# pqpeqr/RL-2048-with-Reinforce-and-Actor-Critic

Hardware: AMD Instinct MI355X
Metric: env steps/sec (whole node) + achieved HBM GB/s, batch=1M 4x4 boards (higher is better)
Workload: dtype u64

## Files before the change

### rl-2048-with-reinforce-and-actor-critic_amd/csrc/g2048.hip

```cpp
#include <hip/hip_runtime.h>

#include <cstdlib>
#include <mutex>
#include <string>

#include "g2048.h"
#include "g2048_core.h"

using namespace g2048;

static_assert(G2048_F_CHANGED == kFChanged && G2048_F_TERMINATED == kFTerminated && G2048_F_TRUNCATED == kFTruncated &&
                  G2048_F_INVALID == kFInvalid && G2048_F_OVERFLOW == kFOverflow,
              "g2048_core.h step flag bits == include/g2048.h");

namespace {

thread_local std::string g_err;
std::mutex g_mu;
constexpr int kMaxDev = 64;
uint8_t* g_tab[kMaxDev] = {};
int g_cus[kMaxDev] = {};

int fail(int code, const std::string& msg) {
    g_err = msg;
    return code;
}

#define G2048_HIP(x)                                                                                  \
    do {                                                                                              \
        hipError_t e_ = (x);                                                                          \
        if (e_ != hipSuccess) return fail(G2048_EHIP, std::string(#x) + ": " + hipGetErrorString(e_)); \
    } while (0)

#ifndef G2048_DIAG
#define G2048_DIAG 0
#endif
#if G2048_DIAG
constexpr int kDiagSlots = 5, kDiagBlocks = 4096;
__device__ uint64_t g_diag_ts[kDiagBlocks * kDiagSlots];
#define G2048_TS(slot)                                                                          \
    do {                                                                                        \
        if (threadIdx.x == 0 && blockIdx.x < kDiagBlocks)                                       \
            g_diag_ts[blockIdx.x * kDiagSlots + (slot)] = __builtin_amdgcn_s_memrealtime();     \
    } while (0)
#else
#define G2048_TS(slot) \
    do {               \
    } while (0)
#endif

constexpr int kBlock = 1024;
constexpr int kLines = 65536;
constexpr int kTabBytes = kLines * 2 + kLines / 2;
constexpr int kTabVec = kTabBytes / 16;
constexpr int kMxOff = kTabBytes;
constexpr int kDevTabBytes = kTabBytes + kLines / 2;
constexpr int kLutSmallN = 16384;
constexpr int64_t kMaxLanesPerLaunch = int64_t(1) << 27;

template <class T>
__device__ __forceinline__ T ld(const T* p, uint32_t idx) {
    return *reinterpret_cast<const T*>(reinterpret_cast<const char*>(p) + idx * (uint32_t)sizeof(T));
}
template <class T>
__device__ __forceinline__ void st(T* p, uint32_t idx, T v) {
    *reinterpret_cast<T*>(reinterpret_cast<char*>(p) + idx * (uint32_t)sizeof(T)) = v;
}

__device__ __forceinline__ void st_obs(float4* base, int q, float4 v) {
    typedef float f4v __attribute__((ext_vector_type(4)));
    __builtin_nontemporal_store(f4v{v.x, v.y, v.z, v.w}, reinterpret_cast<f4v*>(base + q));
}

struct LineFn {
    const uint16_t* line;
    __device__ uint32_t operator()(uint32_t o) const { return line[o]; }
};
struct CodeFn {
    const uint8_t* code;
    __device__ uint32_t operator()(uint32_t o) const { return (code[o >> 1] >> ((o & 1u) << 2)) & 15u; }
};

__device__ inline uint64_t shfl64(uint64_t v, int src) {
    uint32_t lo = (uint32_t)__shfl((int)(uint32_t)v, src, 64);
    uint32_t hi = (uint32_t)__shfl((int)(uint32_t)(v >> 32), src, 64);
    return ((uint64_t)hi << 32) | lo;
}

__device__ inline uint32_t nib(uint64_t b, uint32_t cell) { return (uint32_t)(b >> (4u * cell)) & 15u; }

template <int OBS>
__device__ inline void write_obs_wave(float* __restrict__ obs, uint32_t w0, uint64_t b, uint64_t wmask, int lane,
                                      float scale) {
    if constexpr (OBS == G2048_OBS_ONEHOT) {
        float4* dst = reinterpret_cast<float4*>(obs) + (size_t)w0 * 68;
        const auto value = [&](int q, int src, uint64_t bb) {
            const int j = (q - src * 68) * 4;
            const int c0 = j / 17;
            const int c1 = c0 + 1 < 16 ? c0 + 1 : 15;
            const int p0 = 17 * c0 + (int)nib(bb, c0);
            const int p1 = 17 * c1 + (int)nib(bb, c1);
            float4 v;
            v.x = (j == p0 || j == p1) ? 1.0f : 0.0f;
            v.y = (j + 1 == p0 || j + 1 == p1) ? 1.0f : 0.0f;
            v.z = (j + 2 == p0 || j + 2 == p1) ? 1.0f : 0.0f;
            v.w = (j + 3 == p0 || j + 3 == p1) ? 1.0f : 0.0f;
            return v;
        };
        if (wmask == ~0ull) {
#pragma unroll 4
            for (int k = 0; k < 68; k++) {
                const int q = k * 64 + lane;
                const int src = q / 68;
                st_obs(dst, q, value(q, src, shfl64(b, src)));
            }
        } else {
#pragma unroll 4
            for (int k = 0; k < 68; k++) {
                const int q = k * 64 + lane;
                const int src = q / 68;
                const uint64_t bb = shfl64(b, src);
// ... 72 lines not shown
    g.i_hi = c.y;
    g.has_uint32 = 0u;
    g.uinteger = ld(L.rng_uint, i);
    return g;
}

__device__ inline void store_pcg(const g2048_lanes& L, uint32_t i, const Pcg64& g, bool with_inc) {
    st(reinterpret_cast<ulonglong2*>(L.rng_state), i, make_ulonglong2(g.s_lo, g.s_hi));
    if (with_inc) st(reinterpret_cast<ulonglong2*>(L.rng_inc), i, make_ulonglong2(g.i_lo, g.i_hi));
    st(L.rng_uint, i, g.uinteger);
}

__device__ inline uint32_t fresh_state(const Pcg64& g) {
    return (2u << G2048_LS_MAXT_SHIFT) | G2048_LS_ACTIVE | (g.has_uint32 ? G2048_LS_HAS_U32 : 0u);
}

__device__ inline U4 philox_ctr(uint64_t key, uint64_t seed, uint32_t ctr, uint32_t tag) {
    U4 c{(uint32_t)seed, (uint32_t)(seed >> 32), ctr, tag};
    return philox4x32(c, (uint32_t)key, (uint32_t)(key >> 32));
}

template <int RNG>
__device__ inline uint64_t fresh_board(uint64_t seed, uint64_t key, Pcg64& g) {
    uint64_t b = 0;
    if constexpr (RNG == G2048_RNG_PCG64) {
        g = pcg_seed(seed);
        b = spawn_pcg(b, g);
        b = spawn_pcg(b, g);
    } else {
        const U4 r = philox_ctr(key, seed, 0u, 1u);
        b = spawn_philox(b, U4{r.x, r.y, 0u, 0u});
        b = spawn_philox(b, U4{r.z, r.w, 0u, 0u});
    }
    return b;
}

struct StepArgs {
    g2048_lanes L;
    const uint8_t* actions;
    g2048_step_out out;
    RewardCfg rc;
    float obs_scale;
    int auto_reset;
    int64_t max_steps;
    uint64_t stride, key;
    const uint8_t* tab;
    uint32_t n;
    int diag;
};

template <int OBS, int RNG>
__device__ inline void reset_lane(const StepArgs& a, uint32_t i, uint64_t prev_seed) {
    const g2048_lanes& L = a.L;
    const uint64_t seed = prev_seed + a.stride;
    Pcg64 g;
    g.has_uint32 = 0u;
    const uint64_t b = fresh_board<RNG>(seed, a.key, g);
    st(L.seed, i, seed);
    st(L.board, i, b);
    st(L.state, i, fresh_state(g));
    if constexpr (RNG == G2048_RNG_PCG64) store_pcg(L, i, g, true);
    if (a.out.mask) st(reinterpret_cast<uint32_t*>(a.out.mask), i, mask_word(action_mask(b)));
    if (a.out.mask_bits) st(a.out.mask_bits, i, (uint8_t)action_mask(b));
    if constexpr (OBS != G2048_OBS_NONE)
        if (a.out.obs) write_obs_lane<OBS>(a.out.obs, i, b, a.obs_scale);
}

struct LaneIn {
    uint64_t b, seed;
    uint32_t st, act;
    Pcg64 g;
};

template <int RNG>
__device__ inline void load_lane(const StepArgs& a, uint32_t i, LaneIn& x) {
    const g2048_lanes& L = a.L;
    x.b = ld(L.board, i);
    x.st = ld(L.state, i);
    x.act = ld(a.actions, i);
    if constexpr (RNG == G2048_RNG_PCG64) x.g = load_pcg(L, i);
    else x.seed = ld(L.seed, i);
}

template <int RNG, int XO, int RK>
__device__ inline uint64_t step_lane(const StepArgs& a, uint32_t i, LaneIn& x, const LineFn& lut,
                                     const CodeFn& code, bool& wobs, bool& reset, uint32_t& mbits) {
    static_assert(RK == 0 || XO == 0 || XO == 3, "the lean path writes no score / merged list");
    constexpr bool LIST = XO == 2, EXTRA = XO == 1 || XO == 2;
    const g2048_lanes& L = a.L;
    const uint64_t b = x.b;
    if (EXTRA && a.out.prev_board) st(a.out.prev_board, i, b);
    wobs = false;
    reset = false;
    if (!(x.st & G2048_LS_ACTIVE) || x.act > 3u) {
        st(a.out.reward, i, 0.0f);
        if (EXTRA && a.out.reward64) st(a.out.reward64, i, 0.0);
        st(a.out.flags, i, (uint8_t)((x.st & G2048_LS_ACTIVE) ? G2048_F_BADACTION : G2048_F_INACTIVE));
        if (LIST && a.out.merged) st(a.out.merged, i, 0u);
        if (EXTRA && a.out.score_add) st(a.out.score_add, i, 0u);
        return b;
    }
    const uint32_t sc0 = x.st & G2048_LS_STEP_MASK;
    const uint32_t sc = sc0 + (sc0 < G2048_LS_STEP_MASK ? 1u : 0u);
    uint32_t mt = (x.st >> G2048_LS_MAXT_SHIFT) & 31u;
    if constexpr (RNG == G2048_RNG_PCG64) x.g.has_uint32 = (x.st & G2048_LS_HAS_U32) ? 1u : 0u;

    MoveSummary s;
    uint64_t m, nzm = 0;
    if (G2048_DIAG && (a.diag & 4)) {
        s = MoveSummary{0, 0, 0, 0, 0, 0};
        m = b ^ ((uint64_t)x.act << 60);
        nzm = nz_bits(m);
    } else if constexpr (RK == 1) {
        m = board_move_lean(b, x.act, lut, code, s, nzm);
    } else {
        m = board_move_coded<LIST>(b, x.act, lut, code, s);
    }
    const bool changed = m != b;
    if constexpr (RK == 1) {
        if constexpr (RNG == G2048_RNG_PCG64) {
            if (!(G2048_DIAG && (a.diag & 4))) {
                Pcg64 g2 = x.g;
                uint64_t nzbit;
                const uint64_t m2 = spawn_pcg_lean(m, ~nzm & kNibLsb, g2, nzbit);
                m = changed ? m2 : m;
                nzm = changed ? nzm | nzbit : nzm;
                x.g.s_hi = changed ? g2.s_hi : x.g.s_hi;
                x.g.s_lo = changed ? g2.s_lo : x.g.s_lo;
                x.g.uinteger = changed ? g2.uinteger : x.g.uinteger;
                x.g.has_uint32 = changed ? g2.has_uint32 : x.g.has_uint32;
            }
        } else if (changed && !(G2048_DIAG && (a.diag & 4))) {
            uint64_t nzbit;
            m = spawn_philox_z(m, ~nzm & kNibLsb, philox_ctr(a.key, x.seed, sc, 0u), nzbit);
            nzm |= nzbit;
        }
    } else {
        if (changed && !(G2048_DIAG && (a.diag & 4))) {
            if constexpr (RNG == G2048_RNG_PCG64) m = spawn_pcg(m, x.g);
            else m = spawn_philox(m, philox_ctr(a.key, x.seed, sc, 0u));
        }
        nzm = nz_bits(m);
    }
    const BoardBits bits = board_bits_nz(m, nzm);
    const bool done = bits_done(bits);
    const bool invalid = !changed && !done;
    const double r = env_reward_nz<RK == 1>(a.rc, s, nzm, done, invalid, mt);
    const bool trunc = a.max_steps >= 0 && (int64_t)sc >= a.max_steps && !done;
    const uint32_t fl = (changed ? G2048_F_CHANGED : 0u) | (done ? G2048_F_TERMINATED : 0u) |
                        (trunc ? G2048_F_TRUNCATED : 0u) | (invalid ? G2048_F_INVALID : 0u) |
                        (s.overflow ? G2048_F_OVERFLOW : 0u);
    st(a.out.reward, i, (float)r);
    if (EXTRA && a.out.reward64) st(a.out.reward64, i, r);
    if (LIST && a.out.merged) st(a.out.merged, i, s.list);
    if (EXTRA && a.out.score_add) st(a.out.score_add, i, s.score);
    reset = (done || trunc) && a.auto_reset;
    uint32_t nst = sc | (mt << G2048_LS_MAXT_SHIFT) | ((done || trunc) ? 0u : G2048_LS_ACTIVE);
    if constexpr (RNG == G2048_RNG_PCG64) nst |= x.g.has_uint32 ? G2048_LS_HAS_U32 : 0u;
    st(a.out.flags, i, (uint8_t)(fl | (reset ? G2048_F_RESET : 0u)));
    st(L.board, i, m);
    st(L.state, i, nst);
    if constexpr (RNG == G2048_RNG_PCG64) store_pcg(L, i, x.g, false);
    wobs = true;
    mbits = bits_mask(bits);
    return m;
}

template <int OBS, int RNG, int XO, int RK>
__device__ __forceinline__ void sweep(const StepArgs& a, uint32_t w0, int lane, LaneIn& x, const LineFn& lut,
                                      const CodeFn& code, uint64_t& pending, uint64_t& pseed, uint32_t k) {
    const uint32_t i = w0 + lane;
    bool wobs = false, reset = false;
    uint32_t mbits = 0;
    uint64_t b = 0;
    if (i < a.n) b = step_lane<RNG, XO, RK>(a, i, x, lut, code, wobs, reset, mbits);
    if (reset) {
        if (!pending) {
            if constexpr (RNG == G2048_RNG_PCG64) pseed = ld(a.L.seed, i);
            else pseed = x.seed;
        }
        pending |= 1ull << k;
    }
    if constexpr (XO == 3) {
        if (wobs) st(a.out.mask_bits, i, (uint8_t)mbits);
    } else {
        if (wobs && a.out.mask) st(reinterpret_cast<uint32_t*>(a.out.mask), i, mask_word(mbits));
        if (wobs && a.out.mask_bits) st(a.out.mask_bits, i, (uint8_t)mbits);
    }
    if constexpr (OBS != G2048_OBS_NONE) {
        const uint64_t wm = __ballot(wobs);
        if (G2048_DIAG && (a.diag & 16)) return;
        if (a.out.obs && wm) write_obs_wave<OBS>(a.out.obs, w0, b, wm, lane, a.obs_scale);
    }
}

constexpr int kStepLdsBytes = kTabBytes;
constexpr int kStepLdsVec = kStepLdsBytes / 16;
constexpr int kResetCap = (kStepLdsBytes - 16) / 12;
static_assert(16 + kResetCap * 4 + kResetCap * 8 <= kStepLdsBytes, "reset list fits the LDS area");
static_assert(kTabVec % kBlock == 0, "table fill: whole chunks per thread");

template <int OBS, int RNG, bool LDS, int XO, int U, int RK>
__global__ void __launch_bounds__(kBlock) step_kernel(StepArgs a) {
    static_assert(U == 1, "one board per lane per sweep");
    __shared__ uint4 tab_lds[LDS ? kStepLdsVec : 1];
    const int lane = threadIdx.x & 63;
    const uint32_t w_first = (blockIdx.x * kBlock + threadIdx.x) & ~63u;
    const uint32_t wstride = gridDim.x * kBlock;
    const uint32_t wend = a.n;
    const uint32_t last = a.n - 1u;
    const auto lane_at = [&](uint32_t w) { return w + lane < last ? w + lane : last; };
    G2048_TS(0);
    LaneIn A, B, C;
    uint32_t w0 = w_first, w1 = w_first + wstride;
    load_lane<RNG>(a, lane_at(w0), A);
    load_lane<RNG>(a, lane_at(w1), B);
    const uint8_t* tab = a.tab;
    if constexpr (LDS) {
        const uint4* src = reinterpret_cast<const uint4*>(a.tab);
        if (!(G2048_DIAG && (a.diag & 1))) {
            constexpr uint32_t kChunks = kTabVec / kBlock;
            const uint32_t rot = blockIdx.x % kChunks;
#pragma unroll
            for (uint32_t j = 0; j < kChunks; j++) {
                uint32_t c = j + rot;
                c -= c >= kChunks ? kChunks : 0u;
                const uint32_t k = c * kBlock + threadIdx.x;
                tab_lds[k] = src[k + (RK == 1 && c >= 8u ? (uint32_t)((kMxOff - 2 * kLines) / 16) : 0u)];
            }
        }
        __syncthreads();
        tab = reinterpret_cast<const uint8_t*>(tab_lds);
    }
    G2048_TS(1);
    const LineFn lut{reinterpret_cast<const uint16_t*>(tab)};
    const CodeFn code{tab + (LDS || RK == 0 ? 2 * kLines : kMxOff)};
    uint64_t pending = 0, pseed = 0;
    uint32_t k = 0;
    while (w0 < wend) {
        const uint32_t w2 = w1 + wstride;
        load_lane<RNG>(a, lane_at(w2), C);
        sweep<OBS, RNG, XO, RK>(a, w0, lane, A, lut, code, pending, pseed, k);
        if (w1 >= wend) break;
        const uint32_t w3 = w2 + wstride;
        load_lane<RNG>(a, lane_at(w3), A);
        sweep<OBS, RNG, XO, RK>(a, w1, lane, B, lut, code, pending, pseed, k + 1);
        if (w2 >= wend) break;
        const uint32_t w4 = w3 + wstride;
        load_lane<RNG>(a, lane_at(w4), B);
        sweep<OBS, RNG, XO, RK>(a, w2, lane, C, lut, code, pending, pseed, k + 2);
        w0 = w3;
        w1 = w4;
        k += 3;
    }
    if (G2048_DIAG && (a.diag & 2)) pending = 0;
    if constexpr (LDS) {
        uint32_t* cnt = reinterpret_cast<uint32_t*>(tab_lds);
        uint32_t* ridx = cnt + 4;
        uint64_t* rseed = reinterpret_cast<uint64_t*>(ridx + kResetCap + (kResetCap & 1));
        __syncthreads();
        G2048_TS(2);
        if (threadIdx.x == 0) *cnt = 0u;
        __syncthreads();
        bool first = true;
        while (__ballot(pending != 0ull)) {
            const bool has = pending != 0ull;
            const uint32_t kk = has ? (uint32_t)__builtin_ctzll(pending) : 0u;
            const uint32_t i = w_first + kk * wstride + lane;
            const uint64_t sd = first ? pseed : (has ? ld(a.L.seed, i) : 0ull);
            const uint64_t bal = __ballot(has);
            const int leader = __builtin_ctzll(bal);
            uint32_t base = 0;
            if (lane == leader) base = atomicAdd(cnt, (uint32_t)__popcll(bal));
            base = (uint32_t)__shfl((int)base, leader, 64);
            const uint32_t slot =
                base + __builtin_amdgcn_mbcnt_hi((uint32_t)(bal >> 32), __builtin_amdgcn_mbcnt_lo((uint32_t)bal, 0u));
            if (has) {
                if (slot < (uint32_t)kResetCap) {
                    ridx[slot] = i;
                    rseed[slot] = sd;
                } else {
                    reset_lane<OBS, RNG>(a, i, sd);
                }
                pending &= pending - 1ull;
            }
            first = false;
        }
        __syncthreads();
        G2048_TS(3);
        const uint32_t R = *cnt < (uint32_t)kResetCap ? *cnt : (uint32_t)kResetCap;
        for (uint32_t r = threadIdx.x; r < R; r += kBlock) reset_lane<OBS, RNG>(a, ridx[r], rseed[r]);
    } else {
        bool first = true;
        while (pending) {
            const uint32_t kk = (uint32_t)__builtin_ctzll(pending);
            pending &= pending - 1ull;
            const uint32_t i = w_first + kk * wstride + lane;
            reset_lane<OBS, RNG>(a, i, first ? pseed : ld(a.L.seed, i));
            first = false;
        }
    }
#if G2048_DIAG
    __syncthreads();
    G2048_TS(4);
#endif
}

struct ResetArgs {
    g2048_lanes L;
    const uint64_t* seeds;
    const uint8_t* reset_mask;
    int8_t* mask_out;
    float* obs_out;
    float obs_scale;
    uint64_t key;
    uint32_t n;
};

template <int OBS, int RNG>
__global__ void __launch_bounds__(256) reset_kernel(ResetArgs a) {
    const int lane = threadIdx.x & 63;
    const uint32_t w_first = (blockIdx.x * blockDim.x + threadIdx.x) & ~63u;
    const uint32_t wstride = gridDim.x * blockDim.x;
    for (uint32_t w0 = w_first; w0 < a.n; w0 += wstride) {
        const uint32_t i = w0 + lane;
        bool w = false;
        uint64_t b = 0;
        if (i < a.n && (!a.reset_mask || ld(a.reset_mask, i))) {
            const uint64_t seed = a.seeds ? ld(a.seeds, i) : ld(a.L.seed, i);
            Pcg64 g;
            g.has_uint32 = 0u;
            b = fresh_board<RNG>(seed, a.key, g);
            st(a.L.seed, i, seed);
            st(a.L.board, i, b);
            st(a.L.state, i, fresh_state(g));
            if constexpr (RNG == G2048_RNG_PCG64) store_pcg(a.L, i, g, true);
// ... 502 lines not shown
```

### rl-2048-with-reinforce-and-actor-critic_amd/csrc/g2048_core.h

```cpp
#pragma once
#include <math.h>
#include <stdint.h>

#ifdef __HIPCC__
#define G2048_HD __host__ __device__ inline
#else
#define G2048_HD static inline
#endif

namespace g2048 {

constexpr uint64_t kNibLsb = 0x1111111111111111ull;
constexpr uint64_t kHMask = 0x0111011101110111ull;
constexpr uint64_t kVMask = 0x0000111111111111ull;

G2048_HD int popc64(uint64_t x) { return __builtin_popcountll(x); }

G2048_HD uint64_t nz_bits(uint64_t b) {
    uint64_t x = b | (b >> 1);
    x |= x >> 2;
    return x & kNibLsb;
}

G2048_HD uint64_t transpose(uint64_t x) {
// ... 238 lines not shown
}

G2048_HD uint32_t line_move_alu(uint32_t o, uint32_t& e0, uint32_t& e1) {
    uint32_t out = 0u, sh = 0u, pend = o & 15u;
    e0 = 0u;
    e1 = 0u;
#pragma unroll
    for (int k = 1; k < 4; k++) {
        const uint32_t v = bfe32(o, 4u * k, 4u);
        const bool nz = v != 0u;
        const bool mg = nz && v == pend;
        const uint32_t emit = mg ? (v == 15u ? 15u : v + 1u) : (nz ? pend : 0u);
        out |= emit << sh;
        sh += emit != 0u ? 4u : 0u;
        e1 = (mg && e0 != 0u) ? v + 1u : e1;
        e0 = (mg && e0 == 0u) ? v + 1u : e0;
        pend = mg ? 0u : (nz ? v : pend);
    }
    return out | (pend << sh);
}

template <bool WANT_LIST>
G2048_HD uint64_t board_move_alu(uint64_t b, uint32_t a, MoveSummary& s) {
    const uint64_t mvert = 0ull - (uint64_t)((a == 0u) | (a == 2u));
    const uint64_t mrev = 0ull - (uint64_t)((a == 1u) | (a == 2u));
    const bool back = (a == 0u) | (a == 1u);
    uint64_t f = b ^ ((b ^ transpose(b)) & mvert);
    f ^= (f ^ reverse_rows(f)) & mrev;
    uint32_t e0[4], e1[4];
    uint64_t g = 0;
    uint32_t sum_e = 0, score = 0, max_e = 0, count = 0, list = 0;
#pragma unroll
    for (int j = 0; j < 4; j++) {
        const uint32_t nw = line_move_alu((uint32_t)(f >> (16 * j)) & 0xFFFFu, e0[j], e1[j]);
        g |= (uint64_t)nw << (16 * j);
        score += ((1u << e0[j]) & ~1u) + ((1u << e1[j]) & ~1u);
        sum_e += e0[j] + e1[j];
        max_e = max_e > e0[j] ? max_e : e0[j];
        max_e = max_e > e1[j] ? max_e : e1[j];
    }
    if (WANT_LIST) {
#pragma unroll
        for (int jj = 0; jj < 4; jj++) {
            const uint32_t x0 = back ? e0[3 - jj] : e0[jj], x1 = back ? e1[3 - jj] : e1[jj];
            const uint32_t n0 = x0 != 0u, n1 = x1 != 0u;
            if (n0) list |= ((x0 - 1u) & 15u) << (4u * (count & 7u));
            if (n1) list |= ((x1 - 1u) & 15u) << (4u * ((count + n0) & 7u));
            count += n0 + n1;
        }
    } else {
#pragma unroll
        for (int j = 0; j < 4; j++) count += (e0[j] != 0u) + (e1[j] != 0u);
    }
    s.count = count;
    s.sum_e = sum_e;
    s.score = score;
    s.max_e = max_e;
    s.overflow = max_e >> 4;
    s.list = list;
    g ^= (g ^ reverse_rows(g)) & mrev;
    g ^= (g ^ transpose(g)) & mvert;
    return g;
}

G2048_HD uint32_t line_max_merge_field(uint32_t row) {
    uint32_t e0, e1;
    (void)line_move_alu(row, e0, e1);
    const uint32_t m = e0 > e1 ? e0 : e1;
    return m ? m - 1u : 0u;
}

G2048_HD uint32_t nib_sum64(uint64_t x) {
    const uint64_t t = (x & 0x0F0F0F0F0F0F0F0Full) + ((x >> 4) & 0x0F0F0F0F0F0F0F0Full);
#ifdef __HIP_DEVICE_COMPILE__
    return __builtin_amdgcn_sad_u8((uint32_t)t, 0u, __builtin_amdgcn_sad_u8((uint32_t)(t >> 32), 0u, 0u));
#else
    uint64_t y = t + (t >> 8);
    y += y >> 16;
    y += y >> 32;
    return (uint32_t)(y & 0xFFu);
#endif
}

template <class Lut, class Mx>
G2048_HD uint64_t board_move_lean(uint64_t b, uint32_t a, const Lut& lut, const Mx& mx, MoveSummary& s,
                                  uint64_t& nzg) {
    const uint64_t mvert = 0ull - (uint64_t)((a == 0u) | (a == 2u));
    const uint64_t mrev = 0ull - (uint64_t)((a == 1u) | (a == 2u));
    uint64_t f = b ^ ((b ^ transpose(b)) & mvert);
    f ^= (f ^ reverse_rows(f)) & mrev;
    uint32_t o[4], nw[4], fm[4];
#pragma unroll
    for (int j = 0; j < 4; j++) o[j] = (uint32_t)(f >> (16 * j)) & 0xFFFFu;
#pragma unroll
    for (int j = 0; j < 4; j++) {
        nw[j] = (uint32_t)lut(o[j]);
        fm[j] = (uint32_t)mx(o[j]);
    }
    uint64_t g = 0;
#pragma unroll
    for (int j = 0; j < 4; j++) g |= (uint64_t)nw[j] << (16 * j);
    const uint32_t m01 = fm[0] > fm[1] ? fm[0] : fm[1], m23 = fm[2] > fm[3] ? fm[2] : fm[3];
    const uint32_t mf = m01 > m23 ? m01 : m23;
    g ^= (g ^ reverse_rows(g)) & mrev;
    g ^= (g ^ transpose(g)) & mvert;
    nzg = nz_bits(g);
    s.max_e = mf ? mf + 1u : 0u;
    s.overflow = mf == 15u;
    s.count = (uint32_t)(popc64(nz_bits(b)) - popc64(nzg));
    s.sum_e = nib_sum64(b) - nib_sum64(g) + 2u * s.count;
    if (s.overflow) {
        uint32_t se = 0;
#pragma unroll
        for (int j = 0; j < 4; j++) {
            const LineMerges m = line_merges(o[j], nw[j]);
            se += m.e0 + m.e1;
        }
        s.sum_e = se;
    }
    s.score = 0u;
    s.list = 0u;
    return g;
}

struct BoardBits {
    uint64_t nz, z, eqh, eqv;
};

G2048_HD BoardBits board_bits_nz(uint64_t b, uint64_t nz) {
    BoardBits r;
    r.nz = nz;
    r.z = ~r.nz & kNibLsb;
    r.eqh = ~nz_bits(b ^ (b >> 4)) & r.nz & kHMask;
    r.eqv = ~nz_bits(b ^ (b >> 16)) & r.nz & kVMask;
    return r;
}

G2048_HD BoardBits board_bits(uint64_t b) { return board_bits_nz(b, nz_bits(b)); }

G2048_HD bool bits_done(const BoardBits& r) { return r.z == 0 && (r.eqh | r.eqv) == 0; }

G2048_HD uint32_t bits_mask(const BoardBits& r) {
    uint32_t up = ((r.z & (r.nz >> 16) & kVMask) | r.eqv) != 0;
    uint32_t down = ((r.nz & (r.z >> 16) & kVMask) | r.eqv) != 0;
    uint32_t left = ((r.z & (r.nz >> 4) & kHMask) | r.eqh) != 0;
    uint32_t right = ((r.nz & (r.z >> 4) & kHMask) | r.eqh) != 0;
    return up | (right << 1) | (down << 2) | (left << 3);
}

G2048_HD uint32_t kth_empty_cell(uint64_t zbits, uint32_t k) {
    uint32_t pos = 0;
    uint32_t c = (uint32_t)popc64(zbits & 0xFFFFFFFFull);
    if (k >= c) { k -= c; zbits >>= 32; pos += 32; }
    c = (uint32_t)popc64(zbits & 0xFFFFull);
    if (k >= c) { k -= c; zbits >>= 16; pos += 16; }
    c = (uint32_t)popc64(zbits & 0xFFull);
    if (k >= c) { k -= c; zbits >>= 8; pos += 8; }
    c = (uint32_t)popc64(zbits & 0xFull);
    if (k >= c) { pos += 4; }
    return pos >> 2;
}

struct Pcg64 {
    uint64_t s_lo, s_hi, i_lo, i_hi;
    uint32_t has_uint32, uinteger;
};

constexpr uint64_t kPcgMulHi = 0x2360ED051FC65DA4ull;
constexpr uint64_t kPcgMulLo = 0x4385DF649FCCF645ull;

G2048_HD uint64_t mulhi64(uint64_t a, uint64_t b) { return (uint64_t)(((unsigned __int128)a * b) >> 64); }

G2048_HD void pcg_step(Pcg64& g) {
    uint64_t lo = g.s_lo * kPcgMulLo;
    uint64_t hi = mulhi64(g.s_lo, kPcgMulLo) + g.s_lo * kPcgMulHi + g.s_hi * kPcgMulLo;
    uint64_t nlo = lo + g.i_lo;
    g.s_hi = hi + g.i_hi + (nlo < lo);
    g.s_lo = nlo;
}

G2048_HD uint64_t pcg_next64(Pcg64& g) {
    pcg_step(g);
    uint64_t x = g.s_hi ^ g.s_lo;
    uint32_t rot = (uint32_t)(g.s_hi >> 58);
    return (x >> rot) | (x << ((64u - rot) & 63u));
}

G2048_HD uint32_t pcg_next32(Pcg64& g) {
    if (g.has_uint32) {
        g.has_uint32 = 0;
        return g.uinteger;
    }
    uint64_t v = pcg_next64(g);
    g.has_uint32 = 1;
    g.uinteger = (uint32_t)(v >> 32);
    return (uint32_t)v;
}

G2048_HD double pcg_random(Pcg64& g) { return (double)(pcg_next64(g) >> 11) * (1.0 / 9007199254740992.0); }

G2048_HD uint32_t pcg_bounded(Pcg64& g, uint32_t n) {
    if (n <= 1u) return 0u;
    const uint32_t rng = n - 1u;
    uint64_t m = (uint64_t)pcg_next32(g) * n;
    uint32_t left = (uint32_t)m;
// ... 22 lines not shown

G2048_HD Pcg64 pcg_seed(uint64_t seed) {
    const uint32_t w0 = (uint32_t)seed, w1 = (uint32_t)(seed >> 32);
    const bool two = w1 != 0u;
    uint32_t pool[4];
    uint32_t hc = 0x43b0d7e5u;
    pool[0] = ss_hashmix(w0, hc);
    pool[1] = ss_hashmix(two ? w1 : 0u, hc);
    pool[2] = ss_hashmix(0u, hc);
    pool[3] = ss_hashmix(0u, hc);
#pragma unroll
    for (int s = 0; s < 4; s++)
#pragma unroll
        for (int d = 0; d < 4; d++)
            if (s != d) pool[d] = ss_mix(pool[d], ss_hashmix(pool[s], hc));
    uint32_t w[8];
    uint32_t hb = 0x8b51f9ddu;
#pragma unroll
    for (int i = 0; i < 8; i++) {
        uint32_t v = pool[i & 3];
        v ^= hb;
        hb *= 0x58f38dedu;
        v *= hb;
        v ^= v >> 16;
        w[i] = v;
    }
    const uint64_t st_hi = ((uint64_t)w[1] << 32) | w[0], st_lo = ((uint64_t)w[3] << 32) | w[2];
    const uint64_t sq_hi = ((uint64_t)w[5] << 32) | w[4], sq_lo = ((uint64_t)w[7] << 32) | w[6];
    Pcg64 g;
    g.i_hi = (sq_hi << 1) | (sq_lo >> 63);
    g.i_lo = (sq_lo << 1) | 1u;
    g.s_lo = 0;
    g.s_hi = 0;
    pcg_step(g);
    uint64_t lo = g.s_lo + st_lo;
    g.s_hi = g.s_hi + st_hi + (lo < g.s_lo);
    g.s_lo = lo;
    pcg_step(g);
    g.has_uint32 = 0;
    g.uinteger = 0;
    return g;
}

struct U4 {
    uint32_t x, y, z, w;
};

G2048_HD U4 philox4x32(U4 c, uint32_t k0, uint32_t k1) {
#pragma unroll
    for (int r = 0; r < 10; r++) {
        const uint64_t p0 = (uint64_t)0xD2511F53u * c.x;
        const uint64_t p1 = (uint64_t)0xCD9E8D57u * c.z;
        U4 n;
        n.x = (uint32_t)(p1 >> 32) ^ c.y ^ k0;
        n.y = (uint32_t)p1;
        n.z = (uint32_t)(p0 >> 32) ^ c.w ^ k1;
        n.w = (uint32_t)p0;
        c = n;
        k0 += 0x9E3779B9u;
        k1 += 0xBB67AE85u;
    }
    return c;
}

G2048_HD uint64_t spawn_pcg_z(uint64_t b, uint64_t z, Pcg64& g, uint64_t& nzbit) {
    nzbit = 0;
    uint32_t n = (uint32_t)popc64(z);
    if (n == 0u) return b;
    uint32_t k = pcg_bounded(g, n);
    uint32_t cell = kth_empty_cell(z, k);
    uint64_t e = pcg_random(g) < 0.9 ? 1u : 2u;
    nzbit = 1ull << (4u * cell);
    return b | (e << (4u * cell));
}

G2048_HD uint64_t pcg_output(uint64_t s_hi, uint64_t s_lo) {
    const uint64_t x = s_hi ^ s_lo;
    const uint32_t rot = (uint32_t)(s_hi >> 58);
    return (x >> rot) | (x << ((64u - rot) & 63u));
}

constexpr uint64_t kRandom09 = 8106479329266893ull;

G2048_HD uint64_t spawn_pcg_lean(uint64_t b, uint64_t z, Pcg64& g, uint64_t& nzbit) {
    const uint32_t n = (uint32_t)popc64(z);
    Pcg64 A = g;
    pcg_step(A);
    Pcg64 B = A;
    pcg_step(B);
    const uint64_t oA = pcg_output(A.s_hi, A.s_lo);
    const bool draw = n > 1u;
    const bool fresh = draw && !g.has_uint32;
    const uint32_t u = g.has_uint32 ? g.uinteger : (uint32_t)oA;
    const uint64_t m = (uint64_t)u * n;
    if (draw && (uint32_t)m < n) return spawn_pcg_z(b, z, g, nzbit);
    const uint32_t k = draw ? (uint32_t)(m >> 32) : 0u;
    const uint64_t r_hi = fresh ? B.s_hi : A.s_hi, r_lo = fresh ? B.s_lo : A.s_lo;
    const uint64_t e = (pcg_output(r_hi, r_lo) >> 11) < kRandom09 ? 1u : 2u;
    const uint32_t cell = kth_empty_cell(z, k);
    g.s_hi = r_hi;
    g.s_lo = r_lo;
    g.uinteger = fresh ? (uint32_t)(oA >> 32) : g.uinteger;
    g.has_uint32 = draw ? (g.has_uint32 ^ 1u) : g.has_uint32;
    nzbit = 1ull << (4u * cell);
    return b | (e << (4u * cell));
}

G2048_HD uint64_t spawn_pcg(uint64_t b, Pcg64& g) {
    uint64_t nzbit;
    return spawn_pcg_z(b, ~nz_bits(b) & kNibLsb, g, nzbit);
}

G2048_HD uint32_t softmax_select(const float lg[4], uint32_t mw, bool has_mask, bool greedy, double u, float p[4]) {
    const bool m[4] = {(mw & 0xFFu) != 0u, ((mw >> 8) & 0xFFu) != 0u, ((mw >> 16) & 0xFFu) != 0u, (mw >> 24) != 0u};
    float l[4];
    for (int k = 0; k < 4; k++) l[k] = (!has_mask || m[k]) ? lg[k] : -1e9f;
    const float mx = fmaxf(fmaxf(l[0], l[1]), fmaxf(l[2], l[3]));
    float e[4];
    for (int k = 0; k < 4; k++) e[k] = expf(l[k] - mx);
    const float s = ((e[0] + e[1]) + e[2]) + e[3];
    for (int k = 0; k < 4; k++) p[k] = e[k] / s;
    uint32_t act = 0;
    if (greedy) {
        float best = has_mask ? p[0] * (float)m[0] : p[0];
        for (int k = 1; k < 4; k++) {
            const float q = has_mask ? p[k] * (float)m[k] : p[k];
            if (q > best) {
                best = q;
                act = (uint32_t)k;
            }
        }
    } else {
        double cdf[4], acc = 0.0;
        for (int k = 0; k < 4; k++) {
            acc += (double)p[k];
            cdf[k] = acc;
        }
        for (int k = 0; k < 4; k++) act += (cdf[k] / cdf[3] <= u) ? 1u : 0u;
    }
    return act;
}

G2048_HD uint64_t spawn_philox_z(uint64_t b, uint64_t z, U4 r, uint64_t& nzbit) {
    nzbit = 0;
    uint32_t n = (uint32_t)popc64(z);
    if (n == 0u) return b;
    uint32_t k = (uint32_t)(((uint64_t)r.x * n) >> 32);
    uint32_t cell = kth_empty_cell(z, k);
    uint64_t e = r.y < 3865470566u ? 1u : 2u;
    nzbit = 1ull << (4u * cell);
    return b | (e << (4u * cell));
}

G2048_HD uint64_t spawn_philox(uint64_t b, U4 r) {
    uint64_t nzbit;
    return spawn_philox_z(b, ~nz_bits(b) & kNibLsb, r, nzbit);
}

struct RewardCfg {
    int32_t reward_mode, bonus_mode, use_action_mask;
    uint32_t terms;
    double base_reward_scale, empty_tile_reward, merge_reward, bonus_scale, step_reward, endgame_penalty,
        invalid_action_penalty;
};

constexpr uint32_t kRwInvalidPenalty = 1u, kRwLog2 = 2u, kRwEmpty = 4u, kRwMerge = 8u, kRwEndgame = 16u,
                   kRwBonusRaw = 32u, kRwBonusLog2 = 64u;
G2048_HD uint32_t reward_terms(const RewardCfg& c) {
    return (c.use_action_mask ? 0u : kRwInvalidPenalty) | (c.reward_mode == 0 ? 0u : kRwLog2) |
           (c.empty_tile_reward != 0.0 ? kRwEmpty : 0u) | (c.merge_reward != 0.0 ? kRwMerge : 0u) |
           (c.endgame_penalty != 0.0 ? kRwEndgame : 0u) | (c.bonus_mode == 1 ? kRwBonusRaw : 0u) |
           (c.bonus_mode == 2 ? kRwBonusLog2 : 0u);
}

template <bool LOG2_ONLY = false>
G2048_HD double env_reward_nz(const RewardCfg& c, const MoveSummary& s, uint64_t final_nz, bool done, bool invalid,
                              uint32_t& max_tile_e) {
    uint32_t t = c.terms;
#ifdef __HIP_DEVICE_COMPILE__
    asm volatile("" : "+s"(t));
#endif
    if ((t & kRwInvalidPenalty) && invalid) return c.invalid_action_penalty;
    double r = (LOG2_ONLY || (t & kRwLog2)) ? (double)s.sum_e : (double)s.score;
    r *= c.base_reward_scale;
    if (t & kRwEmpty) {
        const int ne = 16 - popc64(final_nz);
        r += c.empty_tile_reward * (double)ne;
    }
// ... 65 lines not shown
```

Before: 33.65 billion.

## Overlap LDS table fill with table-independent step prefix for first two boards

Splits the lean move and RNG spawn into a table-independent prefix (orientation transform, tile counts, PCG look-ahead or Philox draw) and a table-dependent suffix. In the LDS lean kernel, it issues all table-fill global loads first, computes the prefixes for the first two preloaded boards while those loads are in flight, then writes LDS and syncs. The goal is to hide table-fill latency at kernel start. In exchange it adds register pressure from the carried prefix state, needs inline-asm pins to hold the ordering, and recovers the PCG increment on the rare rejection path.

```diff
diff --git a/rl-2048-with-reinforce-and-actor-critic_amd/csrc/g2048.hip b/rl-2048-with-reinforce-and-actor-critic_amd/csrc/g2048.hip
--- a/rl-2048-with-reinforce-and-actor-critic_amd/csrc/g2048.hip
+++ b/rl-2048-with-reinforce-and-actor-critic_amd/csrc/g2048.hip
@@ -36,7 +36,7 @@
 #define G2048_DIAG 0
 #endif
 #if G2048_DIAG
-constexpr int kDiagSlots = 5, kDiagBlocks = 4096;
+constexpr int kDiagSlots = 6, kDiagBlocks = 4096;
 __device__ uint64_t g_diag_ts[kDiagBlocks * kDiagSlots];
 #define G2048_TS(slot)                                                                          \
     do {                                                                                        \
@@ -275,10 +275,119 @@
     else x.seed = ld(L.seed, i);
 }
 
+__device__ inline uint32_t lane_step_count(uint32_t st) {
+    const uint32_t sc0 = st & G2048_LS_STEP_MASK;
+    return sc0 + (sc0 < G2048_LS_STEP_MASK ? 1u : 0u);
+}
+
+struct LanePre {
+    uint32_t st, act;
+    MoveFrame mv;
+    uint64_t s_lo, s_hi;
+    uint32_t uinteger;
+    PcgAhead ah;
+    uint64_t seed;
+    uint32_t rx, ry;
+    uint64_t b;
+};
+
+template <int RNG>
+__device__ __forceinline__ LanePre lean_prefix(const StepArgs& a, const LaneIn& x) {
+    LanePre p;
+    p.st = x.st;
+    p.act = x.act;
+    p.mv = move_lean_prefix(x.b, x.act);
+    p.b = x.b;
+    if constexpr (RNG == G2048_RNG_PCG64) {
+        p.s_lo = x.g.s_lo;
+        p.s_hi = x.g.s_hi;
+        p.uinteger = x.g.uinteger;
+        p.ah = spawn_pcg_prefix(x.g);
+    } else {
+        p.seed = x.seed;
+        const U4 r = philox_ctr(a.key, x.seed, lane_step_count(x.st), 0u);
+        p.rx = r.x;
+        p.ry = r.y;
+    }
+    return p;
+}
+
+template <int RNG, int XO>
+__device__ __forceinline__ uint64_t lean_suffix(const StepArgs& a, uint32_t i, const LanePre& p, const LineFn& lut,
+                                       const CodeFn& code, bool& wobs, bool& reset, uint32_t& mbits) {
+    static_assert(XO == 0 || XO == 3, "the lean path writes no score / merged list");
+    const g2048_lanes& L = a.L;
+    wobs = false;
+    reset = false;
+    if (!(p.st & G2048_LS_ACTIVE) || p.act > 3u) {
+        st(a.out.reward, i, 0.0f);
+        st(a.out.flags, i, (uint8_t)((p.st & G2048_LS_ACTIVE) ? G2048_F_BADACTION : G2048_F_INACTIVE));
+        return 0ull;
+    }
+    const uint32_t sc = lane_step_count(p.st);
+    uint32_t mt = (p.st >> G2048_LS_MAXT_SHIFT) & 31u;
+    Pcg64 g;
+    if constexpr (RNG == G2048_RNG_PCG64) {
+        g.s_lo = p.s_lo;
+        g.s_hi = p.s_hi;
+        g.uinteger = p.uinteger;
+        g.has_uint32 = (p.st & G2048_LS_HAS_U32) ? 1u : 0u;
+    }
+    MoveSummary s;
+    uint64_t m, nzm = 0;
+    bool changed;
+    const bool nocompute = G2048_DIAG && (a.diag & 4);
+    if (nocompute) {
+        s = MoveSummary{0, 0, 0, 0, 0, 0};
+        m = p.b ^ ((uint64_t)p.act << 60);
+        nzm = nz_bits(m);
+        changed = m != p.b;
+    } else {
+        m = move_lean_suffix(p.mv, p.act, lut, code, s, nzm, changed);
+    }
+    if constexpr (RNG == G2048_RNG_PCG64) {
+        if (!nocompute) {
+            Pcg64 g2 = g;
+            uint64_t nzbit;
+            const uint64_t m2 = spawn_pcg_suffix(m, ~nzm & kNibLsb, g2, p.ah, nzbit);
+            m = changed ? m2 : m;
+            nzm = changed ? nzm | nzbit : nzm;
+            g.s_hi = changed ? g2.s_hi : g.s_hi;
+            g.s_lo = changed ? g2.s_lo : g.s_lo;
+            g.uinteger = changed ? g2.uinteger : g.uinteger;
+            g.has_uint32 = changed ? g2.has_uint32 : g.has_uint32;
+        }
+    } else if (changed && !nocompute) {
+        uint64_t nzbit;
+        m = spawn_philox_z(m, ~nzm & kNibLsb, U4{p.rx, p.ry, 0u, 0u}, nzbit);
+        nzm |= nzbit;
+    }
+    const BoardBits bits = board_bits_nz(m, nzm);
+    const bool done = bits_done(bits);
+    const bool invalid = !changed && !done;
+    const double r = env_reward_nz<true>(a.rc, s, nzm, done, invalid, mt);
+    const bool trunc = a.max_steps >= 0 && (int64_t)sc >= a.max_steps && !done;
+    const uint32_t fl = (changed ? G2048_F_CHANGED : 0u) | (done ? G2048_F_TERMINATED : 0u) |
+                        (trunc ? G2048_F_TRUNCATED : 0u) | (invalid ? G2048_F_INVALID : 0u) |
+                        (s.overflow ? G2048_F_OVERFLOW : 0u);
+    st(a.out.reward, i, (float)r);
+    reset = (done || trunc) && a.auto_reset;
+    uint32_t nst = sc | (mt << G2048_LS_MAXT_SHIFT) | ((done || trunc) ? 0u : G2048_LS_ACTIVE);
+    if constexpr (RNG == G2048_RNG_PCG64) nst |= g.has_uint32 ? G2048_LS_HAS_U32 : 0u;
+    st(a.out.flags, i, (uint8_t)(fl | (reset ? G2048_F_RESET : 0u)));
+    st(L.board, i, m);
+    st(L.state, i, nst);
+    if constexpr (RNG == G2048_RNG_PCG64) store_pcg(L, i, g, false);
+    wobs = true;
+    mbits = bits_mask(bits);
+    return m;
+}
+
 template <int RNG, int XO, int RK>
 __device__ inline uint64_t step_lane(const StepArgs& a, uint32_t i, LaneIn& x, const LineFn& lut,
                                      const CodeFn& code, bool& wobs, bool& reset, uint32_t& mbits) {
     static_assert(RK == 0 || XO == 0 || XO == 3, "the lean path writes no score / merged list");
+    if constexpr (RK == 1) return lean_suffix<RNG, XO>(a, i, lean_prefix<RNG>(a, x), lut, code, wobs, reset, mbits);
     constexpr bool LIST = XO == 2, EXTRA = XO == 1 || XO == 2;
     const g2048_lanes& L = a.L;
     const uint64_t b = x.b;
@@ -293,52 +402,28 @@
         if (EXTRA && a.out.score_add) st(a.out.score_add, i, 0u);
         return b;
     }
-    const uint32_t sc0 = x.st & G2048_LS_STEP_MASK;
-    const uint32_t sc = sc0 + (sc0 < G2048_LS_STEP_MASK ? 1u : 0u);
+    const uint32_t sc = lane_step_count(x.st);
     uint32_t mt = (x.st >> G2048_LS_MAXT_SHIFT) & 31u;
     if constexpr (RNG == G2048_RNG_PCG64) x.g.has_uint32 = (x.st & G2048_LS_HAS_U32) ? 1u : 0u;
 
     MoveSummary s;
-    uint64_t m, nzm = 0;
+    uint64_t m;
     if (G2048_DIAG && (a.diag & 4)) {
         s = MoveSummary{0, 0, 0, 0, 0, 0};
         m = b ^ ((uint64_t)x.act << 60);
-        nzm = nz_bits(m);
-    } else if constexpr (RK == 1) {
-        m = board_move_lean(b, x.act, lut, code, s, nzm);
     } else {
         m = board_move_coded<LIST>(b, x.act, lut, code, s);
     }
     const bool changed = m != b;
-    if constexpr (RK == 1) {
-        if constexpr (RNG == G2048_RNG_PCG64) {
-            if (!(G2048_DIAG && (a.diag & 4))) {
-                Pcg64 g2 = x.g;
-                uint64_t nzbit;
-                const uint64_t m2 = spawn_pcg_lean(m, ~nzm & kNibLsb, g2, nzbit);
-                m = changed ? m2 : m;
-                nzm = changed ? nzm | nzbit : nzm;
-                x.g.s_hi = changed ? g2.s_hi : x.g.s_hi;
-                x.g.s_lo = changed ? g2.s_lo : x.g.s_lo;
-                x.g.uinteger = changed ? g2.uinteger : x.g.uinteger;
-                x.g.has_uint32 = changed ? g2.has_uint32 : x.g.has_uint32;
-            }
-        } else if (changed && !(G2048_DIAG && (a.diag & 4))) {
-            uint64_t nzbit;
-            m = spawn_philox_z(m, ~nzm & kNibLsb, philox_ctr(a.key, x.seed, sc, 0u), nzbit);
-            nzm |= nzbit;
-        }
-    } else {
-        if (changed && !(G2048_DIAG && (a.diag & 4))) {
-            if constexpr (RNG == G2048_RNG_PCG64) m = spawn_pcg(m, x.g);
-            else m = spawn_philox(m, philox_ctr(a.key, x.seed, sc, 0u));
-        }
-        nzm = nz_bits(m);
-    }
+    if (changed && !(G2048_DIAG && (a.diag & 4))) {
+        if constexpr (RNG == G2048_RNG_PCG64) m = spawn_pcg(m, x.g);
+        else m = spawn_philox(m, philox_ctr(a.key, x.seed, sc, 0u));
+    }
+    const uint64_t nzm = nz_bits(m);
     const BoardBits bits = board_bits_nz(m, nzm);
     const bool done = bits_done(bits);
     const bool invalid = !changed && !done;
-    const double r = env_reward_nz<RK == 1>(a.rc, s, nzm, done, invalid, mt);
+    const double r = env_reward_nz<false>(a.rc, s, nzm, done, invalid, mt);
     const bool trunc = a.max_steps >= 0 && (int64_t)sc >= a.max_steps && !done;
     const uint32_t fl = (changed ? G2048_F_CHANGED : 0u) | (done ? G2048_F_TERMINATED : 0u) |
                         (trunc ? G2048_F_TRUNCATED : 0u) | (invalid ? G2048_F_INVALID : 0u) |
@@ -359,18 +444,18 @@
     return m;
 }
 
-template <int OBS, int RNG, int XO, int RK>
-__device__ __forceinline__ void sweep(const StepArgs& a, uint32_t w0, int lane, LaneIn& x, const LineFn& lut,
-                                      const CodeFn& code, uint64_t& pending, uint64_t& pseed, uint32_t k) {
+template <int OBS, int RNG, int XO, class Step>
+__device__ __forceinline__ void sweep_with(const StepArgs& a, uint32_t w0, int lane, uint64_t xseed, const Step& step,
+                                           uint64_t& pending, uint64_t& pseed, uint32_t k) {
     const uint32_t i = w0 + lane;
     bool wobs = false, reset = false;
     uint32_t mbits = 0;
     uint64_t b = 0;
-    if (i < a.n) b = step_lane<RNG, XO, RK>(a, i, x, lut, code, wobs, reset, mbits);
+    if (i < a.n) b = step(i, wobs, reset, mbits);
     if (reset) {
         if (!pending) {
             if constexpr (RNG == G2048_RNG_PCG64) pseed = ld(a.L.seed, i);
-            else pseed = x.seed;
+            else pseed = xseed;
         }
         pending |= 1ull << k;
     }
@@ -387,18 +472,134 @@
     }
 }
 
+template <int OBS, int RNG, int XO, int RK>
+__device__ __forceinline__ void sweep(const StepArgs& a, uint32_t w0, int lane, LaneIn& x, const LineFn& lut,
+                                      const CodeFn& code, uint64_t& pending, uint64_t& pseed, uint32_t k) {
+    uint64_t xseed = 0;
+    if constexpr (RNG != G2048_RNG_PCG64) xseed = x.seed;
+    sweep_with<OBS, RNG, XO>(
+        a, w0, lane, xseed,
+        [&](uint32_t i, bool& wobs, bool& reset, uint32_t& mbits) {
+            return step_lane<RNG, XO, RK>(a, i, x, lut, code, wobs, reset, mbits);
+        },
+        pending, pseed, k);
+}
+
+template <int OBS, int RNG, int XO>
+__device__ __forceinline__ void sweep_suffix(const StepArgs& a, uint32_t w0, int lane, const LanePre& p,
+                                             const LineFn& lut, const CodeFn& code, uint64_t& pending,
+                                             uint64_t& pseed, uint32_t k) {
+    uint64_t xseed = 0;
+    if constexpr (RNG != G2048_RNG_PCG64) xseed = p.seed;
+    sweep_with<OBS, RNG, XO>(
+        a, w0, lane, xseed,
+        [&](uint32_t i, bool& wobs, bool& reset, uint32_t& mbits) {
+            return lean_suffix<RNG, XO>(a, i, p, lut, code, wobs, reset, mbits);
+        },
+        pending, pseed, k);
+}
+
+template <int OBS, int RNG, int XO, int RK, class LaneAt>
+__device__ __forceinline__ void sweep_loop(const StepArgs& a, const LaneAt& lane_at, int lane, uint32_t wstride,
+                                           LaneIn& X, LaneIn& Y, LaneIn& Z, uint32_t w0, uint32_t w1, uint32_t k,
+                                           const LineFn& lut, const CodeFn& code, uint64_t& pending, uint64_t& pseed) {
+    const uint32_t wend = a.n;
+    while (w0 < wend) {
+        const uint32_t w2 = w1 + wstride;
+        load_lane<RNG>(a, lane_at(w2), Z);
+        sweep<OBS, RNG, XO, RK>(a, w0, lane, X, lut, code, pending, pseed, k);
+        if (w1 >= wend) break;
+        const uint32_t w3 = w2 + wstride;
+        load_lane<RNG>(a, lane_at(w3), X);
+        sweep<OBS, RNG, XO, RK>(a, w1, lane, Y, lut, code, pending, pseed, k + 1);
+        if (w2 >= wend) break;
+        const uint32_t w4 = w3 + wstride;
+        load_lane<RNG>(a, lane_at(w4), Y);
+        sweep<OBS, RNG, XO, RK>(a, w2, lane, Z, lut, code, pending, pseed, k + 2);
+        w0 = w3;
+        w1 = w4;
+        k += 3;
+    }
+}
+
 constexpr int kStepLdsBytes = kTabBytes;
 constexpr int kStepLdsVec = kStepLdsBytes / 16;
 constexpr int kResetCap = (kStepLdsBytes - 16) / 12;
 static_assert(16 + kResetCap * 4 + kResetCap * 8 <= kStepLdsBytes, "reset list fits the LDS area");
 static_assert(kTabVec % kBlock == 0, "table fill: whole chunks per thread");
 
+constexpr uint32_t kFillChunks = kTabVec / kBlock;
+static_assert(kFillChunks == 10, "G2048_FILL_EACH lists the chunks");
+#define G2048_FILL_EACH(X) X(0) X(1) X(2) X(3) X(4) X(5) X(6) X(7) X(8) X(9)
+
+__device__ __forceinline__ uint32_t fill_chunk(uint32_t j) {
+    uint32_t c = j + blockIdx.x % kFillChunks;
+    c -= c >= kFillChunks ? kFillChunks : 0u;
+    return c;
+}
+
+template <int RK>
+__device__ __forceinline__ uint4 fill_load(const uint4* src, uint32_t j) {
+    const uint32_t c = fill_chunk(j);
+    const uint4* base = src + (c * kBlock + (RK == 1 && c >= 8u ? (uint32_t)((kMxOff - 2 * kLines) / 16) : 0u));
+    return ld(base, threadIdx.x);
+}
+#define G2048_FILL_ISSUE(J) const uint4 fill##J = fill ? fill_load<RK>(src, J) : uint4{};
+#define G2048_FILL_WRITE(J) if (fill) tab_lds[fill_chunk(J) * kBlock + threadIdx.x] = fill##J;
+
+__device__ __forceinline__ void pin(uint32_t& v) {
+#if defined(__HIP_DEVICE_COMPILE__)
+    asm volatile("" : "+v"(v));
+#else
+    (void)v;
+#endif
+}
+__device__ __forceinline__ void pin(uint64_t& v) {
+    uint32_t lo = (uint32_t)v, hi = (uint32_t)(v >> 32);
+    pin(lo);
+    pin(hi);
+    v = ((uint64_t)hi << 32) | lo;
+}
+
+__device__ __forceinline__ void order_point() { asm volatile("" ::: "memory"); }
+
+template <int RNG>
+__device__ __forceinline__ void pin_in(LaneIn& x) {
+    pin(x.b);
+    pin(x.st);
+    pin(x.act);
+    if constexpr (RNG == G2048_RNG_PCG64) {
+        pin(x.g.s_lo);
+        pin(x.g.s_hi);
+        pin(x.g.i_lo);
+        pin(x.g.i_hi);
+    } else {
+        pin(x.seed);
+    }
+}
+
+template <int RNG>
+__device__ __forceinline__ void pin_pre(LanePre& p) {
+    pin(p.mv.f);
+    pin(p.mv.tiles);
+    if constexpr (RNG == G2048_RNG_PCG64) {
+        pin(p.ah.a_lo);
+        pin(p.ah.a_hi);
+        pin(p.ah.b_lo);
+        pin(p.ah.b_hi);
+        pin(p.ah.oA);
+    } else {
+        pin(p.rx);
+        pin(p.ry);
+    }
+}
+
 template <int OBS, int RNG, bool LDS, int XO, int U, int RK>
 __global__ void __launch_bounds__(kBlock) step_kernel(StepArgs a) {
     static_assert(U == 1, "one board per lane per sweep");
     __shared__ uint4 tab_lds[LDS ? kStepLdsVec : 1];
     const int lane = threadIdx.x & 63;
-    const uint32_t w_first = (blockIdx.x * kBlock + threadIdx.x) & ~63u;
+    const uint32_t w_first = __builtin_amdgcn_readfirstlane((blockIdx.x * kBlock + threadIdx.x) & ~63u);
     const uint32_t wstride = gridDim.x * kBlock;
     const uint32_t wend = a.n;
     const uint32_t last = a.n - 1u;
@@ -409,19 +610,24 @@
     load_lane<RNG>(a, lane_at(w0), A);
     load_lane<RNG>(a, lane_at(w1), B);
     const uint8_t* tab = a.tab;
+    constexpr bool HEAD = LDS && RK == 1;
+    LanePre P0, P1;
     if constexpr (LDS) {
         const uint4* src = reinterpret_cast<const uint4*>(a.tab);
-        if (!(G2048_DIAG && (a.diag & 1))) {
-            constexpr uint32_t kChunks = kTabVec / kBlock;
-            const uint32_t rot = blockIdx.x % kChunks;
-#pragma unroll
-            for (uint32_t j = 0; j < kChunks; j++) {
-                uint32_t c = j + rot;
-                c -= c >= kChunks ? kChunks : 0u;
-                const uint32_t k = c * kBlock + threadIdx.x;
-                tab_lds[k] = src[k + (RK == 1 && c >= 8u ? (uint32_t)((kMxOff - 2 * kLines) / 16) : 0u)];
-            }
-        }
+        const bool fill = !(G2048_DIAG && (a.diag & 1));
+        G2048_FILL_EACH(G2048_FILL_ISSUE)
+        if constexpr (HEAD) {
+            order_point();
+            pin_in<RNG>(A);
+            pin_in<RNG>(B);
+            P0 = lean_prefix<RNG>(a, A);
+            P1 = lean_prefix<RNG>(a, B);
+            pin_pre<RNG>(P0);
+            pin_pre<RNG>(P1);
+            order_point();
+            G2048_TS(5);
+        }
+        G2048_FILL_EACH(G2048_FILL_WRITE)
         __syncthreads();
         tab = reinterpret_cast<const uint8_t*>(tab_lds);
     }
@@ -429,22 +635,20 @@
     const LineFn lut{reinterpret_cast<const uint16_t*>(tab)};
     const CodeFn code{tab + (LDS || RK == 0 ? 2 * kLines : kMxOff)};
     uint64_t pending = 0, pseed = 0;
-    uint32_t k = 0;
-    while (w0 < wend) {
-        const uint32_t w2 = w1 + wstride;
-        load_lane<RNG>(a, lane_at(w2), C);
-        sweep<OBS, RNG, XO, RK>(a, w0, lane, A, lut, code, pending, pseed, k);
-        if (w1 >= wend) break;
-        const uint32_t w3 = w2 + wstride;
-        load_lane<RNG>(a, lane_at(w3), A);
-        sweep<OBS, RNG, XO, RK>(a, w1, lane, B, lut, code, pending, pseed, k + 1);
-        if (w2 >= wend) break;
-        const uint32_t w4 = w3 + wstride;
-        load_lane<RNG>(a, lane_at(w4), B);
-        sweep<OBS, RNG, XO, RK>(a, w2, lane, C, lut, code, pending, pseed, k + 2);
-        w0 = w3;
-        w1 = w4;
-        k += 3;
+    if constexpr (HEAD) {
+        if (w0 < wend) {
+            const uint32_t w2 = w1 + wstride;
+            load_lane<RNG>(a, lane_at(w2), C);
+            sweep_suffix<OBS, RNG, XO>(a, w0, lane, P0, lut, code, pending, pseed, 0u);
+            if (w1 < wend) {
+                const uint32_t w3 = w2 + wstride;
+                load_lane<RNG>(a, lane_at(w3), A);
+                sweep_suffix<OBS, RNG, XO>(a, w1, lane, P1, lut, code, pending, pseed, 1u);
+                sweep_loop<OBS, RNG, XO, RK>(a, lane_at, lane, wstride, C, A, B, w2, w3, 2u, lut, code, pending, pseed);
+            }
+        }
+    } else {
+        sweep_loop<OBS, RNG, XO, RK>(a, lane_at, lane, wstride, A, B, C, w0, w1, 0u, lut, code, pending, pseed);
     }
     if (G2048_DIAG && (a.diag & 2)) pending = 0;
     if constexpr (LDS) {
diff --git a/rl-2048-with-reinforce-and-actor-critic_amd/csrc/g2048_core.h b/rl-2048-with-reinforce-and-actor-critic_amd/csrc/g2048_core.h
--- a/rl-2048-with-reinforce-and-actor-critic_amd/csrc/g2048_core.h
+++ b/rl-2048-with-reinforce-and-actor-critic_amd/csrc/g2048_core.h
@@ -344,13 +344,27 @@
 #endif
 }
 
-template <class Lut, class Mx>
-G2048_HD uint64_t board_move_lean(uint64_t b, uint32_t a, const Lut& lut, const Mx& mx, MoveSummary& s,
-                                  uint64_t& nzg) {
+struct MoveFrame {
+    uint64_t f;
+    uint32_t tiles;
+};
+
+G2048_HD MoveFrame move_lean_prefix(uint64_t b, uint32_t a) {
     const uint64_t mvert = 0ull - (uint64_t)((a == 0u) | (a == 2u));
     const uint64_t mrev = 0ull - (uint64_t)((a == 1u) | (a == 2u));
-    uint64_t f = b ^ ((b ^ transpose(b)) & mvert);
-    f ^= (f ^ reverse_rows(f)) & mrev;
+    MoveFrame p;
+    p.f = b ^ ((b ^ transpose(b)) & mvert);
+    p.f ^= (p.f ^ reverse_rows(p.f)) & mrev;
+    p.tiles = (uint32_t)popc64(nz_bits(b)) | (nib_sum64(b) << 8);
+    return p;
+}
+
+template <class Lut, class Mx>
+G2048_HD uint64_t move_lean_suffix(const MoveFrame& p, uint32_t a, const Lut& lut, const Mx& mx, MoveSummary& s,
+                                   uint64_t& nzg, bool& changed) {
+    const uint64_t mvert = 0ull - (uint64_t)((a == 0u) | (a == 2u));
+    const uint64_t mrev = 0ull - (uint64_t)((a == 1u) | (a == 2u));
+    const uint64_t f = p.f;
     uint32_t o[4], nw[4], fm[4];
 #pragma unroll
     for (int j = 0; j < 4; j++) o[j] = (uint32_t)(f >> (16 * j)) & 0xFFFFu;
@@ -364,13 +378,14 @@
     for (int j = 0; j < 4; j++) g |= (uint64_t)nw[j] << (16 * j);
     const uint32_t m01 = fm[0] > fm[1] ? fm[0] : fm[1], m23 = fm[2] > fm[3] ? fm[2] : fm[3];
     const uint32_t mf = m01 > m23 ? m01 : m23;
+    changed = g != f;
     g ^= (g ^ reverse_rows(g)) & mrev;
     g ^= (g ^ transpose(g)) & mvert;
     nzg = nz_bits(g);
     s.max_e = mf ? mf + 1u : 0u;
     s.overflow = mf == 15u;
-    s.count = (uint32_t)(popc64(nz_bits(b)) - popc64(nzg));
-    s.sum_e = nib_sum64(b) - nib_sum64(g) + 2u * s.count;
+    s.count = (p.tiles & 0xFFu) - (uint32_t)popc64(nzg);
+    s.sum_e = (p.tiles >> 8) - nib_sum64(g) + 2u * s.count;
     if (s.overflow) {
         uint32_t se = 0;
 #pragma unroll
@@ -383,6 +398,13 @@
     s.score = 0u;
     s.list = 0u;
     return g;
+}
+
+template <class Lut, class Mx>
+G2048_HD uint64_t board_move_lean(uint64_t b, uint32_t a, const Lut& lut, const Mx& mx, MoveSummary& s,
+                                  uint64_t& nzg) {
+    bool changed;
+    return move_lean_suffix(move_lean_prefix(b, a), a, lut, mx, s, nzg, changed);
 }
 
 struct BoardBits {
@@ -571,20 +593,39 @@
 
 constexpr uint64_t kRandom09 = 8106479329266893ull;
 
-G2048_HD uint64_t spawn_pcg_lean(uint64_t b, uint64_t z, Pcg64& g, uint64_t& nzbit) {
-    const uint32_t n = (uint32_t)popc64(z);
+struct PcgAhead {
+    uint64_t a_lo, a_hi, b_lo, b_hi;
+    uint64_t oA;
+};
+
+G2048_HD PcgAhead spawn_pcg_prefix(const Pcg64& g) {
     Pcg64 A = g;
     pcg_step(A);
     Pcg64 B = A;
     pcg_step(B);
-    const uint64_t oA = pcg_output(A.s_hi, A.s_lo);
+    return PcgAhead{A.s_lo, A.s_hi, B.s_lo, B.s_hi, pcg_output(A.s_hi, A.s_lo)};
+}
+
+G2048_HD void pcg_recover_inc(Pcg64& g, const PcgAhead& p) {
+    const uint64_t lo = g.s_lo * kPcgMulLo;
+    const uint64_t hi = mulhi64(g.s_lo, kPcgMulLo) + g.s_lo * kPcgMulHi + g.s_hi * kPcgMulLo;
+    g.i_lo = p.a_lo - lo;
+    g.i_hi = p.a_hi - hi - (p.a_lo < lo);
+}
+
+G2048_HD uint64_t spawn_pcg_suffix(uint64_t b, uint64_t z, Pcg64& g, const PcgAhead& p, uint64_t& nzbit) {
+    const uint32_t n = (uint32_t)popc64(z);
+    const uint64_t oA = p.oA;
     const bool draw = n > 1u;
     const bool fresh = draw && !g.has_uint32;
     const uint32_t u = g.has_uint32 ? g.uinteger : (uint32_t)oA;
     const uint64_t m = (uint64_t)u * n;
-    if (draw && (uint32_t)m < n) return spawn_pcg_z(b, z, g, nzbit);
+    if (draw && (uint32_t)m < n) {
+        pcg_recover_inc(g, p);
+        return spawn_pcg_z(b, z, g, nzbit);
+    }
     const uint32_t k = draw ? (uint32_t)(m >> 32) : 0u;
-    const uint64_t r_hi = fresh ? B.s_hi : A.s_hi, r_lo = fresh ? B.s_lo : A.s_lo;
+    const uint64_t r_hi = fresh ? p.b_hi : p.a_hi, r_lo = fresh ? p.b_lo : p.a_lo;
     const uint64_t e = (pcg_output(r_hi, r_lo) >> 11) < kRandom09 ? 1u : 2u;
     const uint32_t cell = kth_empty_cell(z, k);
     g.s_hi = r_hi;
@@ -593,6 +634,10 @@
     g.has_uint32 = draw ? (g.has_uint32 ^ 1u) : g.has_uint32;
     nzbit = 1ull << (4u * cell);
     return b | (e << (4u * cell));
+}
+
+G2048_HD uint64_t spawn_pcg_lean(uint64_t b, uint64_t z, Pcg64& g, uint64_t& nzbit) {
+    return spawn_pcg_suffix(b, z, g, spawn_pcg_prefix(g), nzbit);
 }
 
 G2048_HD uint64_t spawn_pcg(uint64_t b, Pcg64& g) {
```

Measured after the change: 33.57 billion. Within noise of the previous version (-0.2%).
